# Rick0514/SimpleSLAM

Hardware: AMD Instinct MI355X
Metric: scans/s (65 k-pt scan vs 1 M-pt submap, LOAM 10 iters) + pose RMSE vs CPU ref (higher is better)
Workload: dtype f64; 1 GPU; pcr=loam, 65536-pt 64-beam scan vs 1000000-pt submap, 10 GN iters, early exit off, index rebuilt per call (previous call's bounding box and tile layout reused as checked hints), inputs in HBM; parallelism=single GPU, scans_cycled=8

## Files before the change

simpleslam_amd/csrc/loam.hip:

```cpp
#include <hip/hip_ext.h>

#include "pcr_internal.h"
#include "peer_exchange.h"
#include "small_math.h"

namespace pcr {



static constexpr int kNb = 8;
static constexpr uint32_t kNoPos = 0xffffffffu;
static constexpr uint32_t kKeyEmpty = 0xffffffffu;

struct Nb8 {
    double d[kNb];
    uint32_t idx[kNb];
    float x[kNb], y[kNb], z[kNb];
};

__device__ __forceinline__ bool knn_less(double d, uint32_t i, double d2, uint32_t i2) {
    return (d < d2) | ((d == d2) & (i < i2));
}

__device__ __forceinline__ double sqdist(double qx, double qy, double qz, float px, float py, float pz) {
// ... 339 lines not shown
        for (int j = 0; j < 3; ++j) if (perm[i] == j) x[j] = v;
    }
}


struct WaveCand { double d; uint32_t idx, pos; };
static constexpr int kWaveTab = 280;

__device__ __forceinline__ bool knn8_wave(const GridHeader& h, const float4* __restrict__ pts, const uint32_t* __restrict__ cell_start,
                                          double qx, double qy, double qz, double max_sq, double seed_sq, WaveCand* tab, uint32_t pos_out[kNb],
                                          double* next_sq, bool* inside_out) {
    const int lane = threadIdx.x & 63;
#pragma unroll
    for (int j = 0; j < kNb; ++j) pos_out[j] = kNoPos;
    *next_sq = max_sq;
    const double rx = qx - h.origin[0], ry = qy - h.origin[1], rz = qz - h.origin[2];
    const double fx = floor(rx * h.inv_cell), fy = floor(ry * h.inv_cell), fz = floor(rz * h.inv_cell);
    const bool inside = (fx >= 1.0 && fx <= (double)(h.dims[0] - 2) && fy >= 1.0 && fy <= (double)(h.dims[1] - 2) && fz >= 1.0 &&
                         fz <= (double)(h.dims[2] - 2));
    *inside_out = inside;
    if (!inside) return true;
    const int cx = (int)fx, cy = (int)fy, cz = (int)fz;
    uint32_t rs = 0, len = 0;
    if (lane < 9) {
        const uint32_t key = ((uint32_t)(cz + lane / 3 - 1) * (uint32_t)h.dims[1] + (uint32_t)(cy + lane % 3 - 1)) * (uint32_t)h.dims[0] + (uint32_t)cx;
        rs = cell_start[key - 1];
        len = cell_start[key + 2] - rs;
    }
    uint32_t incl = len;
#pragma unroll
    for (int d = 1; d < 16; d <<= 1) { const uint32_t t = __shfl_up(incl, d, 64); if (lane >= d) incl += t; }
    const uint32_t total = __shfl(incl, 8, 64);
    if (total > (uint32_t)kWaveTab) return false;
    uint32_t r_start[9], r_excl[9];
#pragma unroll
    for (int r = 0; r < 9; ++r) { r_start[r] = __shfl(rs, r, 64); r_excl[r] = __shfl(incl - len, r, 64); }
    uint32_t n_in = 0;
    double out_min = max_sq;
    for (uint32_t c0 = 0; c0 < total; c0 += 64) {
        const uint32_t c = c0 + (uint32_t)lane;
        bool in = false;
        WaveCand w; w.d = max_sq; w.idx = 0xffffffffu; w.pos = kNoPos;
        if (c < total) {
            uint32_t pos = 0;
#pragma unroll
            for (int r = 0; r < 9; ++r) if (c >= r_excl[r]) pos = r_start[r] + (c - r_excl[r]);
            const float4 p = pts[pos];
            const double d = sqdist(qx, qy, qz, p.x, p.y, p.z);
            w.d = d; w.idx = __float_as_uint(p.w); w.pos = pos;
            in = d <= seed_sq;
            if (!in) out_min = fmin(out_min, d);
        }
        const unsigned long long m = __ballot(in);
        if (in) tab[n_in + (uint32_t)__popcll(m & ((1ull << lane) - 1ull))] = w;
        n_in += (uint32_t)__popcll(m);
    }
#pragma unroll
    for (int sft = 32; sft >= 1; sft >>= 1) out_min = fmin(out_min, __shfl_xor(out_min, sft, 64));
    __builtin_amdgcn_fence(__ATOMIC_RELEASE, "workgroup");
    for (uint32_t c = lane; c < n_in; c += 64) {
        const WaveCand me = tab[c];
        uint32_t rank = 0;
#pragma unroll 4
        for (uint32_t j = 0; j < n_in; ++j) {
            const WaveCand o = tab[j];
            rank += knn_less(o.d, o.idx, me.d, me.idx) ? 1u : 0u;
        }
        if (rank <= (uint32_t)kNb) { tab[kWaveTab + rank] = me; }
    }
    __builtin_amdgcn_fence(__ATOMIC_RELEASE, "workgroup");
#pragma unroll
    for (int j = 0; j < kNb; ++j) {
        if ((uint32_t)j < n_in) pos_out[j] = tab[kWaveTab + j].pos;
    }
    double nx = out_min;
    if (n_in > (uint32_t)kNb) nx = fmin(nx, tab[kWaveTab + kNb].d);
    *next_sq = fmin(max_sq, nx);
    return true;
}

static constexpr int kRowStride = 258;
static constexpr int kSparseMisses = 8;
struct MissExchange {
    uint32_t count, fallback;
    uint32_t list[256];
    float qx[256], qy[256], qz[256];
    double seed[256];
    union {
        struct {
            uint32_t pos[kNb][256];
            double bound[256];
            uint32_t state[256];
            uint32_t keys[kNb + 1][256];
            uint32_t idmask[256];
        } res;
        double rows[8 * kRowStride];
    } u;
};

struct EntryWrite {
    uint32_t what;
    Nb8 s;
    float q[3];
    double bound_sq;
    double x[3];
    uint32_t flags;
};

__device__ __forceinline__ void entry_store_wave(NnCacheEntry* __restrict__ e0, const EntryWrite& w, float4* stage) {
    const int lane = threadIdx.x & 63;
    if (w.what & 8u) e0[lane].flags = 0;
    float4* const mine = stage + lane * kEntryVec;
#pragma unroll
    for (int j = 0; j < kNb; ++j) mine[j] = make_float4(w.s.x[j], w.s.y[j], w.s.z[j], __uint_as_float(w.s.idx[j]));
    mine[kNb] = make_float4(w.q[0], w.q[1], w.q[2], __double2float_rd(sqrt(w.bound_sq) * (1.0 - 1e-15)));
    union { struct { double x[3]; uint32_t pidx[5]; uint32_t flags; } t; float4 v[3]; } tail;
    tail.t.x[0] = w.x[0]; tail.t.x[1] = w.x[1]; tail.t.x[2] = w.x[2];
#pragma unroll
    for (int j = 0; j < 5; ++j) tail.t.pidx[j] = w.s.idx[j];
    tail.t.flags = w.flags;
#pragma unroll
    for (int f = 0; f < 3; ++f) mine[kNb + 1 + f] = tail.v[f];
    const uint32_t fields = ((w.what & 1u) ? 0x0ffu : 0u) | ((w.what & 2u) ? 0x100u : 0u) | ((w.what & 4u) ? 0xe00u : 0u);
    __builtin_amdgcn_fence(__ATOMIC_RELEASE, "workgroup");
    float4* const dst = reinterpret_cast<float4*>(e0);
#pragma unroll
    for (int i = 0; i < kEntryVec; ++i) {
        const uint32_t c = (uint32_t)(i * 64 + lane);
        const uint32_t owner = c / (uint32_t)kEntryVec, f = c - owner * (uint32_t)kEntryVec;
        const uint32_t m = (uint32_t)__shfl((int)fields, (int)owner, 64);
        const float4 v = stage[c];
        if ((m >> f) & 1u) dst[c] = v;
    }
}

template <int kGroup>
__device__ __forceinline__ int loam_point(const LoamArgs& a, const GridHeader& h, const double* __restrict__ pose,
                                          float sx, float sy, float sz, bool valid, const NnCacheEntry& ce_in, bool have_entry,
                                          KnnRuns& sh, MissExchange& ex, double row[7], uint32_t nn_idx[5], uint32_t qi, int* how,
                                          bool* escaped, EntryWrite& ew, unsigned long long* tl, const bool all_search = false) {
    const double ox = (double)sx, oy = (double)sy, oz = (double)sz;
    const float px = (float)(pose[0] * ox + pose[4] * oy + pose[8] * oz + pose[12] * 1.0);
    const float py = (float)(pose[1] * ox + pose[5] * oy + pose[9] * oz + pose[13] * 1.0);
    const float pz = (float)(pose[2] * ox + pose[6] * oy + pose[10] * oz + pose[14] * 1.0);
    const double qx = (double)px, qy = (double)py, qz = (double)pz;
    const bool in_range = valid;
    bool active = valid && !h.empty && !h.overflow;
    if (a.use_tile) {
        const bool in_tile = qx >= a.tile_lo[0] && qx < a.tile_hi[0] && qy >= a.tile_lo[1] && qy < a.tile_hi[1] &&
                             qz >= a.tile_lo[2] && qz < a.tile_hi[2];
        if (!in_tile) { active = false; valid = false; }
    }
    *escaped = false;
    if (h.clamped && active) {
        const double fx = floor((qx - h.origin[0]) * h.inv_cell), fy = floor((qy - h.origin[1]) * h.inv_cell), fz = floor((qz - h.origin[2]) * h.inv_cell);
        const int cm = h.cut_mask;
        *escaped = ((cm & 1) && fx <= (double)kPad) || ((cm & 8) && fx >= (double)(h.dims[0] - kPad - 1)) ||
                   ((cm & 2) && fy <= (double)kPad) || ((cm & 16) && fy >= (double)(h.dims[1] - kPad - 1)) ||
                   ((cm & 4) && fz <= (double)kPad) || ((cm & 32) && fz >= (double)(h.dims[2] - kPad - 1));
    }
    Nb8 s;
    bool moved = false;
    const bool have_seed = have_entry && active && (ce_in.flags & 1u);
    bool hit = false;
    if (have_seed) hit = knn_from_cache(ce_in, qx, qy, qz, s, &moved);
    const int tid = threadIdx.x;
    const bool miss = active && !hit;
    KnnRanges own_ranges;
    own_ranges.inside = false;
#pragma unroll
    for (int r = 0; r < 9; ++r) { own_ranges.ra[r] = 0u; own_ranges.rb[r] = 0u; }
    if (__any(miss)) knn_ranges_issue(h, a.grid.cell_start, px, py, pz, miss, own_ranges);
    if (!all_search) {
    if (tid == 0) ex.count = 0;
    __syncthreads();
    if (miss) {
        const uint32_t m = atomicAdd(&ex.count, 1u);
        ex.list[m] = (uint32_t)tid;
        ex.qx[tid] = px; ex.qy[tid] = py; ex.qz[tid] = pz;
        double sb = a.c.knn_max_sq;
        if (have_seed) {
            double mx = s.d[0];
#pragma unroll
            for (int j = 1; j < kNb; ++j) mx = fmax(mx, s.d[j]);
            sb = fmin(sb, mx);
        }
        ex.seed[tid] = sb;
    }
    __syncthreads();
    }
    if (tl) tl[2] = wall_clock64();
    bool self = false;
    uint32_t self_pos[kNb], self_state = 0u;
    double self_bound = 0.0;
    {
        const uint32_t n_miss = all_search ? 256u : ex.count;
        bool dense = n_miss > (uint32_t)kSparseMisses;
        if (n_miss && !dense) {
            if (tid == 0) ex.fallback = 0;
            __syncthreads();
            const int wave = tid >> 6;
            WaveCand* tab = reinterpret_cast<WaveCand*>(&sh) + (size_t)wave * (kWaveTab + 16);
            for (uint32_t m = wave; m < n_miss; m += 4) {
                const uint32_t owner = ex.list[m];
                uint32_t rp[kNb];
                double nxt = 0.0;
                bool ins = false;
                const bool done = knn8_wave(h, a.grid.pts, a.grid.cell_start, (double)ex.qx[owner], (double)ex.qy[owner], (double)ex.qz[owner],
                                            a.c.knn_max_sq, ex.seed[owner], tab, rp, &nxt, &ins);
                if (!done) { if ((tid & 63) == 0) ex.fallback = 1; }
                else if ((tid & 63) == 0) {
#pragma unroll
                    for (int j = 0; j < kNb; ++j) ex.u.res.pos[j][owner] = rp[j];
                    ex.u.res.bound[owner] = nxt; ex.u.res.state[owner] = ins ? 2u : 0u;
                }
            }
            __syncthreads();
            dense = ex.fallback != 0;
            __syncthreads();
        }
        if (n_miss > 128u && dense) {
            self = true;
            uint32_t key[kNb + 1], idmask = 0u;
            const float gate_f = __double2float_ru(a.c.knn_max_sq * (1.0 + 1e-5));
            const int rc = knn_scan<kGroup>(h, a.grid.pts, a.grid.cell_start, px, py, pz, gate_f, miss, sh, 0u, 0u, key, &idmask, tl, &own_ranges);
            knn_decode(sh, tid, key, idmask, self_pos);
            self_bound = knn_list_bound(key, idmask);
            self_state = rc == 0 ? 0u : (rc == 2 ? 3u : 1u);
        } else if (n_miss && dense) {
            const uint32_t pl2 = n_miss <= 64u ? 2u : 1u;
            const uint32_t per = 256u >> pl2;
            const uint32_t m = (uint32_t)tid & (per - 1u), part = (uint32_t)tid >> (8u - pl2);
            const bool worker = m < n_miss;
            const uint32_t owner = worker ? ex.list[m] : 0u;
            uint32_t key[kNb + 1], idmask = 0u;
            const float gate_f = __double2float_ru(a.c.knn_max_sq * (1.0 + 1e-5));
            const int rc = knn_scan<kGroup>(h, a.grid.pts, a.grid.cell_start, ex.qx[owner], ex.qy[owner], ex.qz[owner], gate_f, worker, sh, part, pl2, key,
                                            &idmask, tl);
            if (pl2) {
                if (worker && part) {
#pragma unroll
                    for (int j = 0; j <= kNb; ++j) ex.u.res.keys[j][tid] = key[j];
                }
                __syncthreads();
                if (worker && !part) {
                    for (uint32_t q = 1; q < (1u << pl2); ++q) {
                        const uint32_t t2 = m + q * per;
#pragma unroll
                        for (int j = 0; j <= kNb; ++j) {
                            uint32_t t = ex.u.res.keys[j][t2];
#pragma unroll
                            for (int k = 0; k < kNb; ++k) { const uint32_t lo = min(key[k], t), hi = max(key[k], t); key[k] = lo; t = hi; }
                            key[kNb] = min(key[kNb], t);
                        }
                    }
                }
                __syncthreads();
            }
            if (worker && !part) {
                uint32_t rp[kNb];
                knn_decode(sh, tid, key, idmask, rp);
#pragma unroll
                for (int j = 0; j < kNb; ++j) ex.u.res.pos[j][owner] = rp[j];
                ex.u.res.bound[owner] = knn_list_bound(key, idmask);
                ex.u.res.state[owner] = rc == 0 ? 0u : (rc == 2 ? 3u : 1u);
            }
        }
    }
    __syncthreads();
    if (tl) tl[3] = wall_clock64();
    bool searched = hit;
    double bound_sq = 0.0;
    if (miss) {
        uint32_t rp[kNb];
#pragma unroll
        for (int j = 0; j < kNb; ++j) rp[j] = self ? self_pos[j] : ex.u.res.pos[j][tid];
        bound_sq = self ? self_bound : ex.u.res.bound[tid];
        uint32_t state = self ? self_state : ex.u.res.state[tid];
        searched = state != 0u;
        float4 p8[kNb];
#pragma unroll
        for (int j = 0; j < kNb; ++j) p8[j] = a.grid.pts[(searched && rp[j] != kNoPos) ? rp[j] : 0u];
        if (tl) { float t_ = 0.f; for (int j = 0; j < kNb; ++j) t_ += p8[j].x; if (t_ == 1.2345e38f) state = 0u; tl[12] = wall_clock64(); }
#pragma unroll
        for (int j = 0; j < kNb; ++j) nb8_set(s, j, p8[j], searched && state != 3u && rp[j] != kNoPos, qx, qy, qz);
        bool ord = true;
#pragma unroll
        for (int j = 0; j < 4; ++j) ord = ord & !knn_less(s.d[j + 1], s.idx[j + 1], s.d[j], s.idx[j]);
#pragma unroll
        for (int j = 5; j < kNb; ++j) ord = ord & !knn_less(s.d[j], s.idx[j], s.d[4], s.idx[4]);
        if (!__all(ord)) nb8_sort(s);
        const bool proven = state == 2u || (state == 1u && (s.idx[4] == 0xffffffffu ? !(bound_sq < a.c.knn_max_sq) : s.d[4] < bound_sq));
        if (searched && !proven) {
            double nxt;
            uint32_t rp2[kNb];
            knn8_exact(h.origin[0], h.origin[1], h.origin[2], h.inv_cell, (uint32_t)h.dims[0], (uint32_t)h.dims[1], a.grid.pts, a.grid.cell_start, qx, qy, qz,
                       a.c.knn_max_sq, rp2, &nxt);
            for (int j = 0; j < kNb; ++j) nb8_set(s, j, a.grid.pts[rp2[j] != kNoPos ? rp2[j] : 0u], rp2[j] != kNoPos, qx, qy, qz);
            nb8_sort(s);
            bound_sq = nxt;
        }
        bound_sq = fmin(bound_sq, a.c.knn_max_sq);
    }
    if (tl) { if (searched && s.d[4] == 1.2345e300) bound_sq = 0.0; tl[13] = wall_clock64(); }
    __syncthreads();
    *how = hit ? 1 : (miss ? 2 : 0);
    const bool real5 = searched && s.idx[4] != 0xffffffffu;

    double x[3] = {0, 0, 0};
    bool plane_ok = false;
    bool reuse = real5 && have_seed && (ce_in.flags & 2u);
#pragma unroll
    for (int j = 0; j < 5; ++j) reuse = reuse && (s.idx[j] == ce_in.pidx[j]);
    const bool gate_knn = real5 && (s.d[4] < a.c.knn_max_sq);
    double A[5][3];
#pragma unroll
    for (int j = 0; j < 5; ++j) { A[j][0] = (double)s.x[j]; A[j][1] = (double)s.y[j]; A[j][2] = (double)s.z[j]; }
// ... 265 lines not shown
    if ((gridDim.x & 7u) == 0) blk = (blockIdx.x & 7u) * (gridDim.x >> 3) + (blockIdx.x >> 3);
    float4* const sh_pre = reinterpret_cast<float4*>(sh_ov);
    GridHeader h;
    {
        static_assert(sizeof(GridHeader) % 4 == 0, "header copied by words");
        const __attribute__((address_space(4))) uint32_t* const hw = (const __attribute__((address_space(4))) uint32_t*)(uintptr_t)a.grid.hdr;
        uint32_t* const w = reinterpret_cast<uint32_t*>(&h);
#pragma unroll
        for (size_t i = 0; i < sizeof(GridHeader) / 4; ++i) w[i] = hw[i];
    }
    float pre_x = 0.f, pre_y = 0.f, pre_z = 0.f;
    const bool use_cache = k > 0 && nn_cache != nullptr;
    const float4* pre_src = nullptr;
    const uint32_t qpb = 256u;
    {
        const uint32_t q = blk * qpb + (uint32_t)tid;
        const float* sp = a.n_src ? src + (size_t)(q < a.n_src ? q : a.n_src - 1u) * a.src_stride
                                  : reinterpret_cast<const float*>(partials);
        pre_x = sp[0]; pre_y = sp[1]; pre_z = sp[2];
        pre_src = (use_cache && q < a.n_src) ? reinterpret_cast<const float4*>(nn_cache + q) : nullptr;
    }
    if (loam_prologue(hd, head, a, k, sh_sum, &sh_pro, tl, pre_src, use_cache ? sh_pre + (tid & ~63) : nullptr)) {
        asm volatile("s_waitcnt vmcnt(0)" ::: "memory");
        return;
    }
    if (tl) tl[1] = wall_clock64();
    double pose[16];
#pragma unroll
    for (int i = 0; i < 16; ++i) pose[i] = sh_pro.pose[i];

    const int e = tid & 31, ch = tid >> 5;
    int er = 7, ec = 7;
    {
        int q = 0;
#pragma unroll
        for (int r = 0; r < 6; ++r) {
#pragma unroll
            for (int c = r; c < 6; ++c) { if (q == e) { er = r; ec = c; } ++q; }
        }
        if (e >= 21 && e < 27) { er = e - 21; ec = 6; }
    }
    double acc = 0.0;
    uint32_t n_hit = 0, n_search = 0, n_esc = 0;
    for (uint32_t base = blk * qpb; base < a.n_src; base += gridDim.x * qpb) {
        const uint32_t q = base + tid;
        const bool valid = q < a.n_src;
        double row[7] = {0, 0, 0, 0, 0, 0, 0};
        uint32_t nn[5] = {0xffffffffu, 0xffffffffu, 0xffffffffu, 0xffffffffu, 0xffffffffu};
        int how = 0;
        bool esc = false;
        EntryWrite ew;
        float sx = pre_x, sy = pre_y, sz = pre_z;
        union { NnCacheEntry e; float4 v[kEntryVec]; } ce;
        ce.e.flags = 0;
        bool all_search = false;
        if (base == blk * qpb) {
            all_search = sh_pro.big_step != 0;
            if (use_cache) asm volatile("s_waitcnt vmcnt(0)" ::: "memory");
            if (use_cache && valid && !sh_pro.big_step) {
#pragma unroll
                for (int f = 0; f < kEntryVec; ++f) ce.v[f] = sh_pre[f * 256 + tid];
            }
            __syncthreads();
        } else {
            sx = sy = sz = 0.f;
            if (valid) {
                const float* sp = src + (size_t)q * a.src_stride;
                sx = sp[0]; sy = sp[1]; sz = sp[2];
                if (use_cache) ce.e = nn_cache[q];
            }
        }
        const int st = loam_point<kGroup>(a, h, pose, sx, sy, sz, valid, ce.e, use_cache && valid && !all_search, sh_knn, sh_ex, row, nn, q, &how, &esc, ew,
                                          base == blk * qpb ? tl : nullptr, all_search);
        if (valid && (a.dbg_status || a.dbg_nn || a.dbg_rows)) {
            const size_t oi = (size_t)q;
            if (a.dbg_status) a.dbg_status[oi] = (int8_t)st;
            if (a.dbg_nn) { for (int j = 0; j < 5; ++j) a.dbg_nn[oi * 5 + j] = (int32_t)nn[j]; }
            if (a.dbg_rows) { for (int j = 0; j < 7; ++j) a.dbg_rows[oi * 7 + j] = st == 0 ? row[j] : 0.0; }
        }
#pragma unroll
        for (int c = 0; c < 7; ++c) sh_rows[c * kRowStride + tid] = st == 0 ? row[c] : 0.0;
        sh_rows[7 * kRowStride + tid] = st == 0 ? 1.0 : 0.0;
        __syncthreads();
        n_hit += (uint32_t)__popcll(__ballot(how == 1)); n_search += (uint32_t)__popcll(__ballot(how == 2));
        if (h.clamped) n_esc += (uint32_t)__popcll(__ballot(esc));
        if (e < 28) {
            const double* ra = sh_rows + er * kRowStride + ch * 32;
            const double* rb = sh_rows + ec * kRowStride + ch * 32;
#pragma unroll 8
            for (int i = 0; i < 32; ++i) acc += ra[i] * rb[i];
        }
        __syncthreads();
        if (__any(ew.what != 0u)) entry_store_wave(nn_cache + (q - (uint32_t)(tid & 63)), ew, reinterpret_cast<float4*>(sh_ov) + (tid >> 6) * (64 * kEntryVec));
        if (base + gridDim.x * qpb < a.n_src) __syncthreads();
    }
    if (tl) tl[5] = wall_clock64();
    sh_sum[ch * 32 + e] = e < 28 ? acc : 0.0;
    __shared__ uint32_t sh_cnt[12];
    if ((tid & 63) == 0) { sh_cnt[(tid >> 6) * 2] = n_hit; sh_cnt[(tid >> 6) * 2 + 1] = n_search; sh_cnt[8 + (tid >> 6)] = n_esc; }
    __syncthreads();
    if (tid < 32) {
        double v = sh_sum[tid];
#pragma unroll
        for (int c = 1; c < 8; ++c) v += sh_sum[c * 32 + tid];
        if (tid == 28) v = (double)(sh_cnt[0] + sh_cnt[2] + sh_cnt[4] + sh_cnt[6]);
        if (tid == 29) v = (double)(sh_cnt[1] + sh_cnt[3] + sh_cnt[5] + sh_cnt[7]);
        if (tid == kSlotEscapes) v = (double)(sh_cnt[8] + sh_cnt[9] + sh_cnt[10] + sh_cnt[11]);
        partials[((size_t)(k & 1) * kMaxPartials + blockIdx.x) * kAccum + tid] = v;
    }
    if (tl) tl[6] = wall_clock64();
}

__global__ __launch_bounds__(256) void loam_finalize_kernel(const double* const partials, LoamState* const state, const double* const reduced,
                                                            const uint32_t n_partials, const int k, const LoamArgs a) {
    __shared__ double sh_sum[8 * 32];
    __shared__ Prologue sh_pro;
    const LoamHead hd = {partials, state, reduced, n_partials};
    HeadLoads head;
    loam_head_issue(hd, k, head);
    loam_prologue(hd, head, a, k, sh_sum, &sh_pro);
    if (threadIdx.x == 0) {
        double T[16];
        for (int i = 0; i < 16; ++i) T[i] = sh_pro.pose[i];
        t2se3(T);
        const LoamState* cur = &state[k & 1];
        LoamResult* r = a.result;
        for (int i = 0; i < 16; ++i) r->pose[i] = T[i];
        r->converged = cur->converged; r->iters_run = cur->iters_run; r->fail = cur->fail;
        r->grid_overflow = a.grid.hdr->overflow; r->grid_empty = a.grid.hdr->empty; r->grid_cells = a.grid.hdr->n_cells;
        r->grid_stale = a.grid.hdr->stale;
        __threadfence_system();
        __hip_atomic_store(&r->pad, 1, __ATOMIC_RELEASE, __HIP_MEMORY_SCOPE_SYSTEM);
    }
}

__device__ __forceinline__ double loam_fold_own_rows(const LoamArgs& a, int k, int comp, int slice) {
    const int done = a.state[k & 1].done;
    const double* const part0 = a.partials + (size_t)(k & 1) * kMaxPartials * kAccum + comp;
    const uint32_t last = a.n_partials ? a.n_partials - 1u : 0u;
    double pv[32];
#pragma unroll
    for (int u = 0; u < 32; ++u) { const uint32_t b = (uint32_t)slice + 8u * u; pv[u] = part0[(size_t)(b < last ? b : last) * kAccum]; }
    double acc = 0.0;
#pragma unroll
    for (int u = 0; u < 32; ++u) acc += ((uint32_t)slice + 8u * u < a.n_partials) ? pv[u] : 0.0;
    for (uint32_t b = (uint32_t)slice + 256u; b < a.n_partials; b += 8u) acc += part0[(size_t)b * kAccum];
    return done ? 0.0 : acc;
}

__global__ __launch_bounds__(256) void loam_reduce_kernel(const LoamArgs a, const int k, double* __restrict__ out) {
    __shared__ double sh_sum[8 * 32];
    const int t = threadIdx.x, comp = t & 31, slice = t >> 5;
    const double acc = loam_fold_own_rows(a, k, comp, slice);
    sh_sum[slice * 32 + comp] = acc;
    __syncthreads();
    if (t < 32) {
        double v = sh_sum[t];
#pragma unroll
        for (int s = 1; s < 8; ++s) v += sh_sum[s * 32 + t];
        if (t == kSlotRankFail) v = (a.rank_fail || a.grid.hdr->overflow) ? 1.0 : 0.0;
        out[t] = v;
    }
}

__global__ __launch_bounds__(256) void loam_peer_exchange_kernel(const LoamArgs a, const int k, const PeerComm pc, const double seq, double* __restrict__ out) {
    __shared__ double sh_sum[8 * 32];
    const int t = threadIdx.x, comp = t & 31, slice = t >> 5;
    const double acc = loam_fold_own_rows(a, k, comp, slice);
    sh_sum[slice * 32 + comp] = acc;
    __syncthreads();
    double v = 0.0;
    if (t < 32) {
        v = sh_sum[t];
#pragma unroll
        for (int s = 1; s < 8; ++s) v += sh_sum[s * 32 + t];
        if (t == kSlotRankFail) v = (a.rank_fail || a.grid.hdr->overflow) ? 1.0 : 0.0;
// ... 46 lines not shown
```

simpleslam_amd/csrc/pcr_internal.h:

```cpp
#pragma once
#include <hip/hip_runtime.h>
#include <hip/hip_ext.h>
#include <stdint.h>
#include <functional>
#include <string>
#include <vector>

#include <stdlib.h>

#include "../../include/pcr_hip.h"

namespace pcr {

struct GridHeader {
    double origin[3];
    double org[3];
    double cell;
    double inv_cell;
    int32_t dims[3];
    uint32_t n_points;
    uint64_t n_cells;
    int32_t overflow;
    int32_t empty;
    double shift;
    int32_t pcl_mode;
    float inv_leaf_f;
    int32_t min_b[3];
    int32_t too_fine;
    float sum_sq;
    int32_t clamped;
    int32_t cut_mask;
    unsigned long long sum_sq_u;
    int32_t stale;
    int32_t pad2_;
};
__host__ __device__ inline double grid_sum_sq(const GridHeader& h) { return h.sum_sq_u ? (double)h.sum_sq_u : (double)h.sum_sq; }

struct ClampBox { double lo[3], hi[3]; int32_t use, pad_; };

struct HeaderTwin { GridHeader* hdr; GridHeader* mirror; uint64_t capacity; double cell; };

struct GridView {
    const GridHeader* hdr;
    const float4* pts;
    const uint32_t* cell_start;
};

static constexpr int kPad = 2;
static constexpr double kProgressWindow = 1048576.0;
static constexpr int kBBoxBlocks = 256;

struct Pose16 { double m[16]; };

struct LoamState {
    double pose[16];
    int32_t done;
    int32_t converged;
    int32_t iters_run;
    int32_t fail;
};

static constexpr int kAccum = 32;
static constexpr int kSlotRankFail = 30;
static constexpr int kSlotEscapes = 31;
static constexpr int kMaxPartials = 512;
static constexpr int kTimelineSlots = 16;

struct LoamConsts {
    double knn_max_sq, plane_thresh, point_thresh, pos_conv, rot_conv;
    int32_t iters, early_exit;
};

struct LoamResult {
    double pose[16];
    int32_t converged, iters_run, fail, grid_overflow, grid_empty, pad;
    uint64_t grid_cells;
    int32_t grid_stale;
    int32_t progress;
};

struct LoamTrace {
    double JtJ[36];
    double JtE[6];
    double x[6];
    int64_t n;
    int64_t cache_hits, searches;
};

struct NnCacheEntry;

struct LoamArgs {
    const float* src;
    uint32_t n_src;
    uint32_t src_stride;
    GridView grid;
    LoamConsts c;
    double init_pose[16];
    LoamState* state;
    double* partials;
    const double* reduced;
    uint32_t n_partials;
    LoamTrace* trace;
    LoamResult* result;
    int8_t* dbg_status;
    double* dbg_rows;
    int32_t* dbg_nn;
    struct NnCacheEntry* nn_cache;
    int32_t use_tile;
    double tile_lo[3], tile_hi[3];
    int32_t coresident;
    int32_t rank_fail;
    unsigned long long* timeline;
};

struct DeviceBuf {
    void* p = nullptr;
    size_t cap = 0;
    DeviceBuf() = default;
    DeviceBuf(const DeviceBuf&) = delete;
    DeviceBuf& operator=(const DeviceBuf&) = delete;
    ~DeviceBuf() { release(); }
    hipError_t reserve(size_t bytes);
    void release();
    template <class T> T* as() const { return static_cast<T*>(p); }
};

static constexpr int kMaxBins = 8192;
static constexpr int kMaxTileShift = 13;

static constexpr uint32_t kNdtUnprepared = 0xffffffffu;
struct TileTail {
    uint32_t* vox_slot; uint32_t* list; uint32_t* count; uint32_t* count_next;
    int32_t min_points; uint32_t capacity;
    const uint8_t* mask; int32_t mshift;
};
struct BuildFilter {
    std::function<hipError_t()> enqueue_mask;
    const uint8_t* mask = nullptr;
    int mshift = 0;
    bool applied = false;
    bool want_tail = false;
    TileTail tail = {};
    bool tail_applied = false;
};

struct GridIndex {
    DeviceBuf sorted, cell_count, cell_start, block_sums, bbox_partials, header, keys, ranks, ticket;
    DeviceBuf kept;
    DeviceBuf tiled, bin_count, bin_start, tile_sq;
// ... 266 lines not shown
```

simpleslam_amd/pcr.py:

```python
import ctypes as C
import os

import numpy as np

_HERE = os.path.dirname(os.path.abspath(__file__))
LIB_PATH = os.environ.get("PCR_LIB") or os.path.join(_HERE, "lib", "libpcr_hip.so")


class PcrParams(C.Structure):
    _fields_ = [
        ("struct_size", C.c_uint32), ("device", C.c_int32),
        ("loam_iters", C.c_int32), ("loam_early_exit", C.c_int32),
        ("loam_knn_max_sq", C.c_double), ("loam_plane_thresh", C.c_double), ("loam_point_thresh", C.c_double),
        ("loam_pos_conv", C.c_double), ("loam_rot_conv", C.c_double),
        ("ndt_resolution", C.c_double), ("ndt_step_size", C.c_double), ("ndt_outlier_ratio", C.c_double),
        ("ndt_trans_eps", C.c_double), ("ndt_max_iters", C.c_int32), ("ndt_min_points", C.c_int32),
        ("ndt_search", C.c_int32),
        ("vgicp_resolution", C.c_double), ("vgicp_k_corr", C.c_int32), ("vgicp_max_iters", C.c_int32),
        ("vgicp_lm_inner", C.c_int32), ("vgicp_rot_eps", C.c_double), ("vgicp_trans_eps", C.c_double),
        ("vgicp_lm_init_scale", C.c_double), ("vgicp_search", C.c_int32),
        ("record_trace", C.c_int32),
        ("index_no_hints", C.c_int32), ("ndt_evaluate_repeats", C.c_int32), ("loam_disable_cache", C.c_int32), ("record_timeline", C.c_int32),
        ("loam_coresident", C.c_int32), ("loam_clamp_margin_mm", C.c_int32), ("full_target", C.c_int32), ("host_optimiser", C.c_int32),
        ("host_copy_xyz", C.c_int32),
# ... 554 lines not shown
        out = [_cand_dict(c) for c in cands[:nc.value]]
        self.isConverge = bool(conv.value)
        return self.isConverge, out, int(ch.value)

    def relocalizeGlobal(self, src, sc, kf_poses, pose, **params):
        if not isinstance(sc, ScanContext):
            raise TypeError("sc must be a ScanContext")
        p, n, s, dev, _k = _cloud(src)
        gp = global_reloc_params(**params)
        pose_np = np.asarray(pose)
        if pose_np.shape != (4, 4) or pose_np.dtype != np.float64:
            raise ValueError("pose must be a float64 4x4 array (written in place)")
        kf = np.asarray(kf_poses, np.float64)
        if kf.ndim != 3 or kf.shape[1:] != (4, 4):
            raise ValueError("kf_poses must have shape (M, 4, 4)")
        kf_cm = np.ascontiguousarray(kf.transpose(0, 2, 1)).reshape(-1)
        cap = max(gp.places, 0) * max(gp.local.refine_top, 0)
        cands = (GlobalRelocCandidate * max(cap, 1))()
        out_pose = np.zeros(16)
        conv, nc, ch = C.c_int(0), C.c_size_t(0), C.c_size_t(0)
        dp = C.POINTER(C.c_double)
        self._check(self._lib.pcr_relocalize_global(self._h, sc._s, kf_cm.ctypes.data_as(dp), kf.shape[0], p, n, s, dev, C.byref(gp),
                                                    out_pose.ctypes.data_as(dp), C.byref(conv), cands, cap, C.byref(nc), C.byref(ch)))
        pose_np[...] = _pose_out(out_pose)
        out = []
        for g in cands[:nc.value]:
            d = dict(place=int(g.place), sc_dist=g.sc_dist, sc_shift=int(g.sc_shift))
            d.update(_cand_dict(g.c))
            out.append(d)
        self.isConverge = bool(conv.value)
        return self.isConverge, out, int(ch.value)

    def _check(self, rc):
        if rc != 0:
            raise PcrError(self._lib.pcr_last_error(self._h).decode())

    def close(self):
        if getattr(self, "_h", None):
            self._lib.pcr_destroy(self._h)
            self._h = None

    def __del__(self):
        try:
            self.close()
        except Exception:
            pass


class LoamRegister(PointCloudRegister):
    method = "loam"

    def linearize(self, src, pose, per_point=False):
        p, n, s, dev, _k = _cloud(src)
        pc = _pose_in(pose)
        JtJ = np.zeros(36)
        JtE = np.zeros(6)
        cnt = C.c_int64(0)
        status = np.zeros(n, np.int8) if per_point else None
        rows = np.zeros((n, 7)) if per_point else None
        nn = np.zeros((n, 5), np.int32) if per_point else None
        dp = C.POINTER(C.c_double)
        vp = lambda a: a.ctypes.data_as(C.c_void_p) if a is not None else None
        self._check(self._lib.pcr_loam_linearize(self._h, p, n, s, dev, pc.ctypes.data_as(dp), JtJ.ctypes.data_as(dp),
                                                 JtE.ctypes.data_as(dp), C.byref(cnt), vp(status), vp(rows), vp(nn)))
        out = dict(JtJ=JtJ.reshape(6, 6), JtE=JtE, n=int(cnt.value))
        if per_point:
            out.update(status=status, rows=rows, nn=nn)
        return out

    def trace(self):
        it = max(1, self.params.loam_iters)
        JtJ, JtE, n, x = np.zeros((it, 36)), np.zeros((it, 6)), np.zeros(it, np.int64), np.zeros((it, 6))
        k = C.c_int32(0)
        vp = lambda a: a.ctypes.data_as(C.c_void_p)
        self._check(self._lib.pcr_get_trace(self._h, C.byref(k), vp(JtJ), vp(JtE), vp(n), vp(x)))
        k = k.value
        hits, srch = np.zeros(it, np.int64), np.zeros(it, np.int64)
        self._check(self._lib.pcr_get_trace_counts(self._h, vp(hits), vp(srch)))
        return dict(iters_run=k, JtJ=JtJ[:k].reshape(-1, 6, 6), JtE=JtE[:k], n=n[:k], x=x[:k], cache_hits=hits[:k], searches=srch[:k])

    def timeline(self):
        nl, nb = C.c_int(0), C.c_int(0)
        self._check(self._lib.pcr_get_timeline(self._h, None, 0, C.byref(nl), C.byref(nb)))
        raw = np.zeros((nl.value, nb.value, 16), np.uint64)
        self._check(self._lib.pcr_get_timeline(self._h, raw.ctypes.data_as(C.c_void_p), raw.size, C.byref(nl), C.byref(nb)))
        t = raw.astype(np.int64)
        return (t - t[:, :, :1].min(axis=1, keepdims=True)) / 100.0


class NdtRegister(PointCloudRegister):
    method = "ndt"

    def derivatives(self, src, p6, double_hessian=False, device_loop=False, kind=0):
        p, n, s, dev, _k = _cloud(src)
        p6 = np.ascontiguousarray(p6, np.float64).reshape(6)
        if device_loop:
            if double_hessian:
                raise ValueError("device_loop: the double Hessian is a pass of its own, kind=2")
            g, H = np.zeros(6), np.zeros(36)
            sc = C.c_double(0)
            dp = C.POINTER(C.c_double)
            self._check(self._lib.pcr_ndt_pass_sums(self._h, p, n, s, dev, p6.ctypes.data_as(dp), int(kind), C.byref(sc), g.ctypes.data_as(dp),
                                                    H.ctypes.data_as(dp)))
            if kind == 2:
                return dict(hess_d=H.reshape(6, 6))
            return dict(score=sc.value, grad=g) if kind == 1 else dict(score=sc.value, grad=g, hess=H.reshape(6, 6))
        g, H = np.zeros(6), np.zeros(36)
        Hd = np.zeros(36) if double_hessian else None
        sc = C.c_double(0)
        dp = C.POINTER(C.c_double)
        self._check(self._lib.pcr_ndt_derivatives(self._h, p, n, s, dev, p6.ctypes.data_as(dp), C.byref(sc), g.ctypes.data_as(dp),
                                                  H.ctypes.data_as(dp), Hd.ctypes.data_as(dp) if Hd is not None else None))
        out = dict(score=sc.value, grad=g, hess=H.reshape(6, 6))
        if double_hessian:
            out["hess_d"] = Hd.reshape(6, 6)
        return out

    def voxels(self):
        cnt, rej = C.c_size_t(0), C.c_size_t(0)
        self._check(self._lib.pcr_ndt_voxels(self._h, None, 0, C.byref(cnt), C.byref(rej)))
        rec = np.dtype([("ijk", np.int32, 3), ("n", np.int32), ("mean", np.float64, 3), ("icov", np.float64, (3, 3))])
        assert rec.itemsize == 112
        raw = np.zeros(cnt.value, rec)
        if cnt.value:
            self._check(self._lib.pcr_ndt_voxels(self._h, raw.ctypes.data_as(C.c_void_p), raw.size, C.byref(cnt), C.byref(rej)))
        raw = raw[np.lexsort((raw["ijk"][:, 2], raw["ijk"][:, 1], raw["ijk"][:, 0]))]
        return dict(ijk=raw["ijk"].copy(), n=raw["n"].copy(), mean=raw["mean"].copy(), icov=raw["icov"].copy(), rejected=int(rej.value))


class VgicpRegister(PointCloudRegister):
    method = "vgicp"

    def correspondences(self):
        cnt = C.c_size_t(0)
        self._check(self._lib.pcr_vgicp_correspondences(self._h, None, 0, C.byref(cnt)))
        rec = np.dtype([("row", np.int32), ("ijk", np.int32, 3)])
        assert rec.itemsize == 16
        raw = np.zeros(cnt.value, rec)
        if cnt.value:
            self._check(self._lib.pcr_vgicp_correspondences(self._h, raw.ctypes.data_as(C.c_void_p), raw.size, C.byref(cnt)))
        return dict(row=raw["row"].copy(), ijk=raw["ijk"].copy())

    def voxels(self):
        cnt = C.c_size_t(0)
        self._check(self._lib.pcr_vgicp_voxels(self._h, None, 0, C.byref(cnt)))
        rec = np.dtype([("ijk", np.int32, 3), ("n", np.int32), ("mean", np.float64, 3), ("cov6", np.float64, 6)])
        assert rec.itemsize == 88
        raw = np.zeros(cnt.value, rec)
        if cnt.value:
            self._check(self._lib.pcr_vgicp_voxels(self._h, raw.ctypes.data_as(C.c_void_p), raw.size, C.byref(cnt)))
        raw = raw[np.lexsort((raw["ijk"][:, 2], raw["ijk"][:, 1], raw["ijk"][:, 0]))]
        cov = raw["cov6"][:, [0, 1, 2, 1, 3, 4, 2, 4, 5]].reshape(-1, 3, 3)
        return dict(ijk=raw["ijk"].copy(), n=raw["n"].copy(), mean=raw["mean"].copy(), cov=cov.copy())

    def initForLC(self):
        self.set_params(vgicp_max_iters=100, vgicp_trans_eps=1e-6)

    def covariances(self, pts):
        p, n, s, dev, _k = _cloud(pts)
        c6 = np.zeros((n, 6))
        self._check(self._lib.pcr_vgicp_covariances(self._h, p, n, s, dev, c6.ctypes.data_as(C.c_void_p)))
        out = np.zeros((n, 3, 3))
        out[:, 0, 0], out[:, 0, 1], out[:, 0, 2], out[:, 1, 1], out[:, 1, 2], out[:, 2, 2] = c6.T
        out[:, 1, 0], out[:, 2, 0], out[:, 2, 1] = out[:, 0, 1], out[:, 0, 2], out[:, 1, 2]
        return out

    def neighbours(self, n):
# ... 344 lines not shown
```

Measured before the change: 4128 scans/s.

## Replace atomic miss list with per-wave ballot compaction and vectorise row sums

Miss compaction now uses a per-wave ballot and mbcnt in place of a shared atomic counter, removing one block barrier and the LDS atomics. Owners are looked up through per-wave prefix counts. The 28-entry JtJ chunk sums read two doubles per LDS load. Cache-entry writes go straight to global memory per lane when few lanes write, skipping the LDS staging. Extra timeline slots are also added for profiling, which costs more branches and registers and makes the list lookup a little more complex.

After: 4192 scans/s (median of 6 runs). +1.6%, better.

```diff
diff --git a/simpleslam_amd/csrc/loam.hip b/simpleslam_amd/csrc/loam.hip
--- a/simpleslam_amd/csrc/loam.hip
+++ b/simpleslam_amd/csrc/loam.hip
@@ -445,11 +445,12 @@
 static constexpr int kRowStride = 258;
 static constexpr int kSparseMisses = 8;
 struct MissExchange {
-    uint32_t count, fallback;
+    uint32_t wcount[4];
+    uint32_t fallback, pad_[3];
     uint32_t list[256];
     float qx[256], qy[256], qz[256];
     double seed[256];
-    union {
+    union alignas(16) {
         struct {
             uint32_t pos[kNb][256];
             double bound[256];
@@ -460,6 +461,15 @@
         double rows[8 * kRowStride];
     } u;
 };
+static_assert(offsetof(MissExchange, u) % 16 == 0 && (kRowStride * sizeof(double)) % 16 == 0 && sizeof(KnnRuns) % 16 == 0,
+              "the chunk sums read two doubles of a row per instruction");
+
+__device__ __forceinline__ uint32_t posted_owner(const MissExchange& ex, const uint32_t c[4], uint32_t m) {
+    const uint32_t p1 = c[0], p2 = p1 + c[1], p3 = p2 + c[2];
+    const uint32_t w = (m >= p1 ? 1u : 0u) + (m >= p2 ? 1u : 0u) + (m >= p3 ? 1u : 0u);
+    const uint32_t first = w == 0u ? 0u : (w == 1u ? p1 : (w == 2u ? p2 : p3));
+    return ex.list[w * 64u + (m - first)];
+}
 
 struct EntryWrite {
     uint32_t what;
@@ -470,21 +480,38 @@
     uint32_t flags;
 };
 
+__device__ __forceinline__ uint32_t entry_fields(const EntryWrite& w, float4 v[kEntryVec]) {
+#pragma unroll
+    for (int j = 0; j < kNb; ++j) v[j] = make_float4(w.s.x[j], w.s.y[j], w.s.z[j], __uint_as_float(w.s.idx[j]));
+    v[kNb] = make_float4(w.q[0], w.q[1], w.q[2], __double2float_rd(sqrt(w.bound_sq) * (1.0 - 1e-15)));
+    union { struct { double x[3]; uint32_t pidx[5]; uint32_t flags; } t; float4 v[3]; } tail;
+    tail.t.x[0] = w.x[0]; tail.t.x[1] = w.x[1]; tail.t.x[2] = w.x[2];
+#pragma unroll
+    for (int j = 0; j < 5; ++j) tail.t.pidx[j] = w.s.idx[j];
+    tail.t.flags = w.flags;
+#pragma unroll
+    for (int f = 0; f < 3; ++f) v[kNb + 1 + f] = tail.v[f];
+    return ((w.what & 1u) ? 0x0ffu : 0u) | ((w.what & 2u) ? 0x100u : 0u) | ((w.what & 4u) ? 0xe00u : 0u);
+}
+
+static constexpr int kFewWriters = 8;
+__device__ __forceinline__ void entry_store_lane(NnCacheEntry* __restrict__ mine_e, const EntryWrite& w) {
+    if (w.what & 8u) mine_e->flags = 0;
+    float4 v[kEntryVec];
+    const uint32_t fields = entry_fields(w, v);
+    float4* const dst = reinterpret_cast<float4*>(mine_e);
+#pragma unroll
+    for (int f = 0; f < kEntryVec; ++f) if ((fields >> f) & 1u) dst[f] = v[f];
+}
+
 __device__ __forceinline__ void entry_store_wave(NnCacheEntry* __restrict__ e0, const EntryWrite& w, float4* stage) {
     const int lane = threadIdx.x & 63;
     if (w.what & 8u) e0[lane].flags = 0;
     float4* const mine = stage + lane * kEntryVec;
-#pragma unroll
-    for (int j = 0; j < kNb; ++j) mine[j] = make_float4(w.s.x[j], w.s.y[j], w.s.z[j], __uint_as_float(w.s.idx[j]));
-    mine[kNb] = make_float4(w.q[0], w.q[1], w.q[2], __double2float_rd(sqrt(w.bound_sq) * (1.0 - 1e-15)));
-    union { struct { double x[3]; uint32_t pidx[5]; uint32_t flags; } t; float4 v[3]; } tail;
-    tail.t.x[0] = w.x[0]; tail.t.x[1] = w.x[1]; tail.t.x[2] = w.x[2];
-#pragma unroll
-    for (int j = 0; j < 5; ++j) tail.t.pidx[j] = w.s.idx[j];
-    tail.t.flags = w.flags;
-#pragma unroll
-    for (int f = 0; f < 3; ++f) mine[kNb + 1 + f] = tail.v[f];
-    const uint32_t fields = ((w.what & 1u) ? 0x0ffu : 0u) | ((w.what & 2u) ? 0x100u : 0u) | ((w.what & 4u) ? 0xe00u : 0u);
+    float4 mv[kEntryVec];
+    const uint32_t fields = entry_fields(w, mv);
+#pragma unroll
+    for (int f = 0; f < kEntryVec; ++f) mine[f] = mv[f];
     __builtin_amdgcn_fence(__ATOMIC_RELEASE, "workgroup");
     float4* const dst = reinterpret_cast<float4*>(e0);
 #pragma unroll
@@ -526,7 +553,9 @@
     bool moved = false;
     const bool have_seed = have_entry && active && (ce_in.flags & 1u);
     bool hit = false;
+    if (tl) { if (px + py + pz == 1.2345e38f) moved = true; tl[16] = wall_clock64(); }
     if (have_seed) hit = knn_from_cache(ce_in, qx, qy, qz, s, &moved);
+    if (tl) { if (hit && s.d[4] == 1.2345e300) moved = true; tl[17] = wall_clock64(); }
     const int tid = threadIdx.x;
     const bool miss = active && !hit;
     KnnRanges own_ranges;
@@ -534,12 +563,12 @@
 #pragma unroll
     for (int r = 0; r < 9; ++r) { own_ranges.ra[r] = 0u; own_ranges.rb[r] = 0u; }
     if (__any(miss)) knn_ranges_issue(h, a.grid.cell_start, px, py, pz, miss, own_ranges);
+    uint32_t posted[4] = {0u, 0u, 0u, 0u};
     if (!all_search) {
-    if (tid == 0) ex.count = 0;
-    __syncthreads();
+    const unsigned long long mb = __ballot(miss);
+    if ((tid & 63) == 0) ex.wcount[tid >> 6] = (uint32_t)__popcll(mb);
     if (miss) {
-        const uint32_t m = atomicAdd(&ex.count, 1u);
-        ex.list[m] = (uint32_t)tid;
+        ex.list[(uint32_t)(tid & ~63) + __builtin_amdgcn_mbcnt_hi((uint32_t)(mb >> 32), __builtin_amdgcn_mbcnt_lo((uint32_t)mb, 0u))] = (uint32_t)tid;
         ex.qx[tid] = px; ex.qy[tid] = py; ex.qz[tid] = pz;
         double sb = a.c.knn_max_sq;
         if (have_seed) {
@@ -551,13 +580,15 @@
         ex.seed[tid] = sb;
     }
     __syncthreads();
-    }
-    if (tl) tl[2] = wall_clock64();
+#pragma unroll
+    for (int wv = 0; wv < 4; ++wv) posted[wv] = ex.wcount[wv];
+    }
+    if (tl) { if (posted[0] == 0x12345678u) moved = true; tl[2] = wall_clock64(); }
     bool self = false;
     uint32_t self_pos[kNb], self_state = 0u;
     double self_bound = 0.0;
     {
-        const uint32_t n_miss = all_search ? 256u : ex.count;
+        const uint32_t n_miss = all_search ? 256u : posted[0] + posted[1] + posted[2] + posted[3];
         bool dense = n_miss > (uint32_t)kSparseMisses;
         if (n_miss && !dense) {
             if (tid == 0) ex.fallback = 0;
@@ -565,7 +596,7 @@
             const int wave = tid >> 6;
             WaveCand* tab = reinterpret_cast<WaveCand*>(&sh) + (size_t)wave * (kWaveTab + 16);
             for (uint32_t m = wave; m < n_miss; m += 4) {
-                const uint32_t owner = ex.list[m];
+                const uint32_t owner = posted_owner(ex, posted, m);
                 uint32_t rp[kNb];
                 double nxt = 0.0;
                 bool ins = false;
@@ -595,7 +626,7 @@
             const uint32_t per = 256u >> pl2;
             const uint32_t m = (uint32_t)tid & (per - 1u), part = (uint32_t)tid >> (8u - pl2);
             const bool worker = m < n_miss;
-            const uint32_t owner = worker ? ex.list[m] : 0u;
+            const uint32_t owner = worker ? posted_owner(ex, posted, m) : 0u;
             uint32_t key[kNb + 1], idmask = 0u;
             const float gate_f = __double2float_ru(a.c.knn_max_sq * (1.0 + 1e-5));
             const int rc = knn_scan<kGroup>(h, a.grid.pts, a.grid.cell_start, ex.qx[owner], ex.qy[owner], ex.qz[owner], gate_f, worker, sh, part, pl2, key,
@@ -1027,16 +1058,26 @@
         for (int c = 0; c < 7; ++c) sh_rows[c * kRowStride + tid] = st == 0 ? row[c] : 0.0;
         sh_rows[7 * kRowStride + tid] = st == 0 ? 1.0 : 0.0;
         __syncthreads();
+        if (tl && base == blk * qpb) tl[18] = wall_clock64();
         n_hit += (uint32_t)__popcll(__ballot(how == 1)); n_search += (uint32_t)__popcll(__ballot(how == 2));
         if (h.clamped) n_esc += (uint32_t)__popcll(__ballot(esc));
         if (e < 28) {
-            const double* ra = sh_rows + er * kRowStride + ch * 32;
-            const double* rb = sh_rows + ec * kRowStride + ch * 32;
+            const double2* ra = reinterpret_cast<const double2*>(sh_rows + er * kRowStride + ch * 32);
+            const double2* rb = reinterpret_cast<const double2*>(sh_rows + ec * kRowStride + ch * 32);
 #pragma unroll 8
-            for (int i = 0; i < 32; ++i) acc += ra[i] * rb[i];
-        }
+            for (int i = 0; i < 16; ++i) {
+                const double2 va = ra[i], vb = rb[i];
+                acc += va.x * vb.x;
+                acc += va.y * vb.y;
+            }
+        }
+        if (tl && base == blk * qpb) { if (acc == 1.2345e300) n_hit = 0u; tl[19] = wall_clock64(); }
         __syncthreads();
-        if (__any(ew.what != 0u)) entry_store_wave(nn_cache + (q - (uint32_t)(tid & 63)), ew, reinterpret_cast<float4*>(sh_ov) + (tid >> 6) * (64 * kEntryVec));
+        const int writers = __popcll(__ballot(ew.what != 0u));
+        if (writers) {
+            if (writers > kFewWriters) entry_store_wave(nn_cache + (q - (uint32_t)(tid & 63)), ew, reinterpret_cast<float4*>(sh_ov) + (tid >> 6) * (64 * kEntryVec));
+            else entry_store_lane(nn_cache + q, ew);
+        }
         if (base + gridDim.x * qpb < a.n_src) __syncthreads();
     }
     if (tl) tl[5] = wall_clock64();
diff --git a/simpleslam_amd/csrc/pcr_internal.h b/simpleslam_amd/csrc/pcr_internal.h
--- a/simpleslam_amd/csrc/pcr_internal.h
+++ b/simpleslam_amd/csrc/pcr_internal.h
@@ -64,7 +64,7 @@
 static constexpr int kSlotRankFail = 30;
 static constexpr int kSlotEscapes = 31;
 static constexpr int kMaxPartials = 512;
-static constexpr int kTimelineSlots = 16;
+static constexpr int kTimelineSlots = 24;
 
 struct LoamConsts {
     double knn_max_sq, plane_thresh, point_thresh, pos_conv, rot_conv;
diff --git a/simpleslam_amd/pcr.py b/simpleslam_amd/pcr.py
--- a/simpleslam_amd/pcr.py
+++ b/simpleslam_amd/pcr.py
@@ -660,7 +660,7 @@
     def timeline(self):
         nl, nb = C.c_int(0), C.c_int(0)
         self._check(self._lib.pcr_get_timeline(self._h, None, 0, C.byref(nl), C.byref(nb)))
-        raw = np.zeros((nl.value, nb.value, 16), np.uint64)
+        raw = np.zeros((nl.value, nb.value, 24), np.uint64)
         self._check(self._lib.pcr_get_timeline(self._h, raw.ctypes.data_as(C.c_void_p), raw.size, C.byref(nl), C.byref(nb)))
         t = raw.astype(np.int64)
         return (t - t[:, :, :1].min(axis=1, keepdims=True)) / 100.0
```
